# carefree0910/carefree-learn

Measured on AMD Instinct MI355X. Metric: train samples/sec + step ms, ViT-B/16 bf16 DDP at 1/2/4/8 MI355X, higher is better.
Workload: dtype bf16

## Files before the change

### __graft_entry__.py

```python
import os
import subprocess
import sys

ROOT = os.path.dirname(os.path.abspath(__file__))
if ROOT not in sys.path:
    sys.path.insert(0, ROOT)

CSRC = os.path.join(ROOT, "carefree-learn_amd", "csrc")
SOURCES = ["errors", "gemm", "gemm_grouped", "attn", "attn_wide", "attn_probs", "norm", "elementwise", "conv", "conv_grouped", "groupnorm", "embed", "random", "tabular", "comm", "sample", "lora", "vq", "conv_direct"]


def build() -> None:
    out_dir = os.path.join(ROOT, "carefree-learn_amd", "_build")
    os.makedirs(out_dir, exist_ok=True)
    hipcc = os.environ.get("HIPCC", "hipcc")
    flags = ["--offload-arch=gfx950", "-O3", "-std=c++17", "-fPIC", "-munsafe-fp-atomics"]
    procs = []
    for name in SOURCES:
        cmd = [hipcc, *flags, "-c", os.path.join(CSRC, name + ".hip"), "-o", os.path.join(out_dir, name + ".o")]
        procs.append((name, subprocess.Popen(cmd, cwd=CSRC)))
    for name, p in procs:
        if p.wait() != 0:
            raise RuntimeError(f"hipcc failed on {name}.hip")
    lib = os.path.join(ROOT, "carefree-learn_amd", "libcfhip.so")
# ... 57 lines not shown
```

### carefree-learn_amd/csrc/gemm.hip

```cpp
#include "gemm_device.h"

namespace {

template <bool AT, bool BT, class C>
struct ItemCtx {
  int m0, n0, z, klen, nk, tile_n;
  __amdgpu_buffer_rsrc_t a_rsrc, b_rsrc;
  StagePlan<C::A_INSTR> pa;
  StagePlan<C::B_INSTR> pb;
  unsigned yx[C::A_INSTR];
  int bshift[C::B_INSTR];
  int btap[C::B_INSTR];
  int kb;
};

template <bool AT, bool BT, class C, int CONV = 0>
__device__ __forceinline__ ItemCtx<AT, BT, C> setup_item(const GemmParams& p, int item, int wave, int lane) {
  ItemCtx<AT, BT, C> c;
  const int ntiles = p.tiles_m * p.tiles_n;
  c.z = item / ntiles;
  const int tile = item - c.z * ntiles;
  int tile_m;
  if (p.group_n > 0) {
    const int per_group = p.group_n * p.tiles_m;
// ... 612 lines not shown
  static const char* const cfg_names[NUM_CFG] = {
      "Cfg<128, 128, 2, 2, 2, 64>", "Cfg<128, 128, 2, 2, 2, 32>", "Cfg<128, 128, 2, 2, 3, 32>", "Cfg<128, 64, 2, 2, 2, 64>",
      "Cfg<128, 128, 2, 2, 4, 32>", "Cfg<128, 64, 2, 2, 2, 32>", "Cfg<128, 64, 2, 2, 3, 32>", "Cfg<256, 256, 2, 4, 4, 32>",
      "Cfg<256, 128, 2, 4, 3, 32>", "Cfg<256, 128, 2, 2, 3, 32>", "Cfg<128, 256, 2, 2, 3, 32>", "Cfg<256, 128, 2, 4, 6, 32>",
      "Cfg<256, 256, 2, 4, 5, 32>", "Cfg<256, 256, 2, 4, 2, 64>", "Cfg<192, 128, 2, 4, 2, 64>", "Cfg<192, 128, 2, 2, 2, 64>",
      "Cfg<128, 256, 2, 4, 2, 64>"};
  int epi = epilogue == CFHIP_EPI_QGELU ? CFHIP_EPI_GELU : epilogue == CFHIP_EPI_DQGELU ? CFHIP_EPI_DGELU : epilogue;
  int cfg = pick_config(M, N, a_trans, b_trans);
  cfg = resolve_config(cfg, a_trans, epi, false);
  const bool phase = cfg >= 7 && cfg <= 12;
  snprintf(out, out_bytes, "%s<%s, %s, %d, %s>", phase ? "gemm_bf16_phase_kernel" : "gemm_bf16_kernel",
           a_trans ? "true" : "false", b_trans ? "true" : "false", epi, cfg_names[cfg]);
  return CFHIP_OK;
}

extern "C" int cfhip_gemm_bf16(const void* A, const void* B, void* C, const float* bias,
                               const void* aux_in, void* aux_out, int M, int N, int K, int64_t lda,
                               int64_t ldb, int64_t ldc, int a_trans, int b_trans, int epilogue,
                               int out_dtype, int accumulate, int split_k, void* workspace,
                               size_t workspace_bytes, float* bias_grad, int bias_grad_accumulate,
                               void* stream) {
  CFHIP_REQUIRE(A && B && C, "gemm: null operand");
  CFHIP_REQUIRE(bias_grad == nullptr || (a_trans && b_trans),
                "gemm: the fused bias gradient exists for layout (1,1) only");
  CFHIP_REQUIRE(M > 0 && N > 0 && K > 0, "gemm: empty problem M=%d N=%d K=%d", M, N, K);
  CFHIP_REQUIRE(epilogue >= 0 && epilogue <= 5, "gemm: bad epilogue %d", epilogue);
  const int quick = epilogue == CFHIP_EPI_QGELU || epilogue == CFHIP_EPI_DQGELU;
  if (epilogue == CFHIP_EPI_QGELU) epilogue = CFHIP_EPI_GELU;
  if (epilogue == CFHIP_EPI_DQGELU) epilogue = CFHIP_EPI_DGELU;
  CFHIP_REQUIRE(!(epilogue == CFHIP_EPI_RESIDUAL || epilogue == CFHIP_EPI_DGELU) || aux_in,
                "gemm: epilogue %d needs aux_in", epilogue);
  CFHIP_REQUIRE(!accumulate || (out_dtype == 1 && epilogue == CFHIP_EPI_NONE), "gemm: accumulate needs f32 output and epilogue NONE");
  CFHIP_REQUIRE(!(epilogue == CFHIP_EPI_GELU || epilogue == CFHIP_EPI_DGELU) || out_dtype == 0,
                "gemm: the GELU / GELU' epilogues write bf16");
  CFHIP_REQUIRE(!(a_trans && !b_trans), "gemm: layout (a_trans=1, b_trans=0) is not provided");
  if (split_k < 1) split_k = 1;
// ... 45 lines not shown
    const int per = (steps + split_k - 1) / split_k;
    split_k = (steps + per - 1) / per;
    p.k_chunk = per * BK_MAX;
  }
  if (split_k > 1) {
    const size_t need = (size_t)split_k * M * N * sizeof(float) + (bias_grad ? (size_t)split_k * M * sizeof(float) : 0);
    if (workspace == nullptr || workspace_bytes < need) {
      cfhip_set_error("gemm: split_k=%d needs %zu workspace bytes, got %zu", split_k, need, workspace_bytes);
      return CFHIP_ERR_WORKSPACE;
    }
    p.slabs = reinterpret_cast<float*>(workspace);
    if (bias_grad) p.bgrad_slabs = p.slabs + (size_t)split_k * M * N;
  }

  int rc;
  int cfg = pick_config(M, N, a_trans, b_trans);
  cfg = resolve_config(cfg, a_trans, epilogue, bias_grad != nullptr);
  switch (cfg) {
    case 1: rc = launch_layout<CfgB>(p, a_trans, b_trans, epilogue, split_k, s); break;
    case 2: rc = launch_layout<CfgC>(p, a_trans, b_trans, epilogue, split_k, s); break;
    case 3: rc = launch_layout<CfgD>(p, a_trans, b_trans, epilogue, split_k, s); break;
    case 4: rc = launch_layout<CfgE>(p, a_trans, b_trans, epilogue, split_k, s); break;
    case 5: rc = launch_layout<CfgF>(p, a_trans, b_trans, epilogue, split_k, s); break;
    case 6: rc = launch_layout<CfgG>(p, a_trans, b_trans, epilogue, split_k, s); break;
    case 7: rc = launch_layout<CfgP, true>(p, a_trans, b_trans, epilogue, split_k, s); break;
    case 8: rc = launch_layout<CfgQ, true>(p, a_trans, b_trans, epilogue, split_k, s); break;
    case 9: rc = launch_layout<CfgR, true>(p, a_trans, b_trans, epilogue, split_k, s); break;
    case 10: rc = launch_layout<CfgS, true>(p, a_trans, b_trans, epilogue, split_k, s); break;
    case 11: rc = launch_layout<CfgT, true>(p, a_trans, b_trans, epilogue, split_k, s); break;
    case 12: rc = launch_layout<CfgU, true>(p, a_trans, b_trans, epilogue, split_k, s); break;
    case 13: rc = launch_layout<CfgW>(p, a_trans, b_trans, epilogue, split_k, s); break;
// ... 2 lines not shown
    case 16: rc = launch_layout<CfgV>(p, a_trans, b_trans, epilogue, split_k, s); break;
    default: rc = launch_layout<CfgA>(p, a_trans, b_trans, epilogue, split_k, s); break;
  }
  if (rc != CFHIP_OK) return rc;
  CFHIP_CHECK_LAUNCH("gemm_bf16");

  if (split_k > 1) {
    const long total = (long)M * (N / 4);
    int blocks = (int)((total + 255) / 256);
    if (blocks > 2048) blocks = 2048;
    hipLaunchKernelGGL(splitk_reduce_kernel, dim3(blocks), dim3(256), 0, s, p.slabs, C, bias, M, N,
                       (long)ldc, split_k, out_dtype, accumulate, p.bgrad_slabs, p.bgrad, p.bgrad_acc);
    CFHIP_CHECK_LAUNCH("splitk_reduce");
  }
  return CFHIP_OK;
}

template <class C, bool PIPE>
static int launch_conv(GemmParams p, int split_k, hipStream_t s) {
  p.tiles_m = (p.M + C::BM - 1) / C::BM;
  p.tiles_n = (p.N + C::BN - 1) / C::BN;
  p.splits = split_k;
  return launch_cfg<false, false, CFHIP_EPI_NONE, C, PIPE, 1>(p, dim3(p.tiles_m * p.tiles_n * split_k), s);
}

struct ConvPlan { int form, split; };

static int conv_split_for(long tiles, long slots, int Cin) {
  const int steps = (9 * Cin + BK_MAX - 1) / BK_MAX;
  if (tiles * 2 > slots || steps < 16) return 1;
// ... 161 lines not shown
```

### carefree-learn_amd/fused.py

```python
import os
from typing import Any, Optional

import torch
from torch import Tensor
from torch.autograd import Function

from . import functional as _functional
from . import ops
from .functional import SideStream, bf16, f32, claim_grads, claim_grads_one_flag, commit_grads, shadow_bf16


FUSE_BIAS_GRAD = True
_SKIP_BIAS_GRAD = False


def _dw_db(w: Tensor, b: Optional[Tensor], dy2: Tensor, x2: Tensor) -> None:
    n, k = w.shape[0], x2.shape[1]
    split = ops.pick_split_k(n, k, x2.shape[0])
    prms = [w] + ([b] if (b is not None and b.requires_grad) else [])
    (gw, acc_w), *bias_claim = claim_grads(prms)
    kw = {}
    if bias_claim:
        gb, acc_b = bias_claim[0]
        if _SKIP_BIAS_GRAD:
# ... 161 lines not shown
        commit_grads((w, b), notify)
        return dx

    if not SPLIT_LN_BWD:
        return param_grads(True)
    SideStream.run(param_grads, (dy2, x2, mean, rstd), lane=1)
    dx, _, _ = ops.layernorm_bwd(dy2, x2, gamma, mean, rstd, dx_add=dx_add, want_param_grads=False, dx_out=dx_out,
                                 dx_add_lo=dx_add_lo, dx_lo_out=dx_lo_out)
    return dx


FWD_HALVES = int(os.environ.get("CFHIP_FWD_HALVES", "2"))


def _block_fwd(x2: Tensor, prm: tuple, num_heads: int, eps1: float, eps2: float, bsz: int, t: int,
               keep_mask: Optional[Tensor], causal: bool, quick: bool = False, streams: Optional[list] = None):
    ln1_w, ln1_b, in_w, qkv_b, out_w, out_b, ln2_w, ln2_b, w1, b1, w2, b2 = prm
    d = x2.shape[1]
    fb = lambda p: None if p is None else p.detach().reshape(-1)
    in_w16, out_w16 = shadow_bf16(in_w), shadow_bf16(out_w)
    w1_16, w2_16 = shadow_bf16(w1), shadow_bf16(w2)
    m, dev = bsz * t, x2.device
    ff = w1.shape[0]
    E = lambda *shape, dt=bf16: torch.empty(shape, dtype=dt, device=dev)
    ln1, mean1, rstd1 = E(m, d), E(m, dt=f32), E(m, dt=f32)
    qkv, o2, lse = E(m, 3 * d), E(m, d), E(bsz, num_heads, t, dt=f32)
    x1 = E(m, d, dt=x2.dtype)
    ln2, mean2, rstd2 = E(m, d), E(m, dt=f32), E(m, dt=f32)
    pre, h, y = E(m, ff), E(m, ff), E(m, d, dt=x2.dtype)
    act = ops.EPI_QGELU if quick else ops.EPI_GELU
    g1, bt1, g2, bt2 = ln1_w.detach(), ln1_b.detach(), ln2_w.detach(), ln2_b.detach()

    def run(b0: int, b1_: int) -> None:
        r = slice(b0 * t, b1_ * t)
        nb = b1_ - b0
        km = None if keep_mask is None else keep_mask[b0:b1_] if keep_mask.shape[0] == bsz else keep_mask
        ops.layernorm_fwd(x2[r], g1, bt1, eps1, out=ln1[r], mean=mean1[r], rstd=rstd1[r])
        ops.gemm(ln1[r], in_w16, bias=fb(qkv_b), out=qkv[r])
        q3 = qkv[r].view(nb, t, 3 * d)
        ops.attn_fwd(q3[..., :d], q3[..., d:2 * d], q3[..., 2 * d:], num_heads, mask=km, causal=causal,
                     out=o2[r].view(nb, t, d), lse=lse[b0:b1_])
        ops.gemm(o2[r], out_w16, bias=fb(out_b), epilogue=ops.EPI_RESIDUAL, aux_in=x2[r], out=x1[r])
        ops.layernorm_fwd(x1[r], g2, bt2, eps2, out=ln2[r], mean=mean2[r], rstd=rstd2[r])
        ops.gemm(ln2[r], w1_16, bias=fb(b1), epilogue=act, aux_out=pre[r], out=h[r])
        ops.gemm(h[r], w2_16, bias=fb(b2), epilogue=ops.EPI_RESIDUAL, aux_in=x1[r], out=y[r])

    if not streams or len(streams) == 1 or bsz < 2 * len(streams):
        run(0, bsz)
    else:
        n = len(streams)
        cuts = _slice_cuts(bsz, n)
        for i, st in enumerate(streams):
            with _functional.on_stream(st):
                run(cuts[i], cuts[i + 1])
    saved = (x2, mean1, rstd1, ln1, qkv, o2, lse, x1, mean2, rstd2, ln2, pre, h, in_w16, out_w16, w1_16, w2_16)
    return y, saved
# ... 3 lines not shown

FIRST_SLICE_SHARE = 0.5


def _slice_cuts(bsz: int, n: int) -> list:
    if n == 2 and FIRST_SLICE_SHARE != 0.5:
        first = min(bsz - 1, max(1, int(round(bsz * FIRST_SLICE_SHARE))))
        return [0, first, bsz]
    return [bsz * i // n for i in range(n + 1)]


BWD_HALVES = int(os.environ.get("CFHIP_BWD_HALVES", "2"))
SideStream.lanes = min(4, max(SideStream.lanes, BWD_HALVES, FWD_HALVES - 1))


def _block_bwd(saved: tuple, prm: tuple, num_heads: int, bsz: int, t: int, keep_mask: Optional[Tensor],
               causal: bool, d2: Tensor, quick: bool = False, streams: Optional[list] = None) -> Tensor:
    x2, mean1, rstd1, ln1, qkv, o2, lse, x1, mean2, rstd2, ln2, pre, h, in_w16, out_w16, w1_16, w2_16 = saved
    ln1_w, ln1_b, in_w, qkv_b, out_w, out_b, ln2_w, ln2_b, w1, b1, w2, b2 = prm
    two = d2.dim() == 3
    d2_full = d2
    d2, d2_lo = (d2[0], d2[1]) if two else (d2, None)
    d = d2.shape[1]
    m = bsz * t
    E = lambda cols: torch.empty((m, cols), dtype=bf16, device=d2.device)
    dpre, dqkv = E(pre.shape[1]), E(3 * d)
    if two:
        dx1_full, dx_full = (torch.empty((2, m, d), dtype=bf16, device=d2.device) for _ in range(2))
        (dx1, dx1_lo), (dx, dx_lo) = (dx1_full[0], dx1_full[1]), (dx_full[0], dx_full[1])
    else:
        dx1, dx = E(d), E(d)
        dx1_lo = dx_lo = None
# ... 14 lines not shown
        km = None if keep_mask is None else keep_mask[b0:b1_] if keep_mask.shape[0] == bsz else keep_mask
        cur = _functional.cur_stream() if d2.is_cuda else None

        def ln(which: int, dy_, x_, w_, b_, mean_, rstd_, add_, out_, add_lo_=None, out_lo_=None) -> None:
            if _ln_defers(w_, b_, dy_):
                _ln_bwd(dy_, x_, w_, b_, mean_, rstd_, dx_add=add_, dx_out=out_, notify=last, dx_add_lo=add_lo_, dx_lo_out=out_lo_)
                return
            if ln_done[which] is not None:
                _functional.rec_wait_event(cur, ln_done[which])
            _ln_bwd(dy_, x_, w_, b_, mean_, rstd_, dx_add=add_, dx_out=out_, notify=last, dx_add_lo=add_lo_, dx_lo_out=out_lo_)
            if nsl > 1 and not last:
                ev = torch.cuda.Event()
                _functional.rec_record_event(ev, cur)
                ln_done[which] = ev

        ops.gemm(d2[r], w2_16, b_trans=True, epilogue=dact, aux_in=pre[r], out=dpre[r])
        dln2 = ops.gemm(dpre[r], w1_16, b_trans=True)
        ln(0, dln2, x1[r], ln2_w, ln2_b, mean2[r], rstd2[r], d2[r], dx1[r], None if d2_lo is None else d2_lo[r],
           None if dx1_lo is None else dx1_lo[r])
        d_o = ops.gemm(dx1[r], out_w16, b_trans=True)
        q3, dq3 = qkv3[b0:b1_], dqkv3[b0:b1_]
        ops.attn_bwd(q3[..., :d], q3[..., d:2 * d], q3[..., 2 * d:], o3[b0:b1_], d_o.view(nb, t, d), lse[b0:b1_], num_heads,
                     dq=dq3[..., :d], dk=dq3[..., d:2 * d], dv=dq3[..., 2 * d:], mask=km, causal=causal)
        dln1 = ops.gemm(dqkv[r], in_w16, b_trans=True)
        ln(1, dln1, x2[r], ln1_w, ln1_b, mean1[r], rstd1[r], dx1[r], dx[r], None if dx1_lo is None else dx1_lo[r],
           None if dx_lo is None else dx_lo[r])

    if nsl == 1:
        run(0)
    else:
        for i, st in enumerate(streams):
            with _functional.on_stream(st):
                run(i)
    _queue_dw(w2, b2, d2, h)
    _queue_dw(w1, b1, dpre, ln2)
    _queue_dw(out_w, out_b, dx1, o2)
    _queue_dw(in_w, qkv_b, dqkv, ln1)
    if two:
        SideStream.keep.append(d2_full)
    return dx_full


GRAD_STREAM_WORDS = int(os.environ.get("CFHIP_GRAD_STREAM_WORDS", "2"))


def _as_bf16_rows(dy: Tensor, rows: int, d: int, words: int = 1) -> Tensor:
    if words == 2:
        out = torch.empty((2, rows, d), dtype=bf16, device=dy.device)
        if dy.dtype == bf16:
            out[0].copy_(dy.contiguous().view(rows, d))
            out[1].zero_()
        else:
            ops.split_f32(dy.float().contiguous().view(rows, d), out[0], out[1])
        return out
    if dy.dtype != bf16:
        dy = ops.to_bf16(dy.float().contiguous())
    return dy.contiguous().view(rows, d)

# ... 166 lines not shown
    n_fresh = n = 0
    fp = 0
    for p in params:
        if p is None:
            continue
        g = p.grad
        if g is None or not p.requires_grad:
            return None
        n += 1
        n_fresh += 1 if getattr(p, "_cfhip_fresh", False) else 0
        fp = (fp * 1000003 + p.data_ptr() + 31 * g.data_ptr()) & 0xFFFFFFFFFFFFFFFF
    state = 1 if n_fresh == n else 0 if n_fresh == 0 else None
    return None if state is None else (state, fp)


def _plan_for(x: Tensor, metas: tuple, keep_mask: Optional[Tensor], causal: bool, params: tuple, training: bool) -> Optional[StackPlan]:
    from . import _lib

    if (not STACK_PLANS or not x.is_cuda or not training or ops.GEMM_TIMER is not None or ops.FLOP_COUNTER is not None
            or _lib.RECORDER is not None or torch.cuda.is_current_stream_capturing() or params[2] is None):
        return None
    state = _grad_state(params)
    if state is None:
        return None
    key = (tuple(x.shape), x.dtype, metas, causal, None if keep_mask is None else keep_mask.data_ptr(), FWD_HALVES, BWD_HALVES,
           DW_GROUP_BLOCKS, DW_GROUP_TILES, DW_TAIL_BLOCKS, DW_PEROP_TAIL, LN_REDUCE_ASIDE, DW_GROUP_ON_MAIN, FIRST_SLICE_SHARE, FUSE_BIAS_GRAD,
           ops.FORCE_SPLIT_K, tuple(id(cb) for cb in _functional.grad_ready_callbacks), x.requires_grad, GRAD_STREAM_WORDS, state)
    pid = id(params[0])
    plan = _plans.get(pid)
    if plan is None or plan.key != key or (plan.params_ref and plan.params_ref[0]() is not params[0]):
        if len(_plans) >= _PLAN_CACHE:
            _plan_conflicts.pop(next(iter(_plans)), None)
            _plans.pop(next(iter(_plans)))
        if plan is not None and plan.params_ref and plan.params_ref[0]() is not params[0]:
            _plan_conflicts.pop(pid, None)
        plan = _plans[pid] = StackPlan(key, params)
    return plan


class MixingStackFn(Function):

    @staticmethod
# ... 1 lines not shown
        m0 = metas[0]
        return int(m0[4]) if len(m0) > 4 and m0[4] else default

    @staticmethod
    def _slices_bwd(metas: tuple, default: int) -> int:
        m0 = metas[0]
        return int(m0[5]) if len(m0) > 5 and m0[5] else MixingStackFn._slices(metas, default)

    @staticmethod
    def _words(metas: tuple, x_is_f32: bool) -> int:
        m0 = metas[0]
        w = int(m0[6]) if len(m0) > 6 and m0[6] else GRAD_STREAM_WORDS
        return 2 if (w == 2 and x_is_f32) else 1

    @staticmethod
    def _forward_body(cur: Tensor, bsz: int, t: int, metas: tuple, keep_mask: Optional[Tensor], causal: bool, params: tuple):
        nblk = len(metas)
        all_saved = []
        streams = None
        FWD_HALVES = MixingStackFn._slices(metas, globals()["FWD_HALVES"])
        if FWD_HALVES > 1 and cur.is_cuda and bsz >= 2 * FWD_HALVES:
            for i in range(nblk):
                for j in (2, 4, 8, 10):
                    shadow_bf16(params[12 * i + j])
            main = _functional.cur_stream()
            streams = [main] + [SideStream.fork(lane) for lane in range(FWD_HALVES - 1)]
            if any(st is None for st in streams):
                streams = None
        for i, meta in enumerate(metas):
            num_heads, eps1, eps2 = meta[:3]
            quick = bool(meta[3]) if len(meta) > 3 else False
            cur, saved = _block_fwd(cur, params[12 * i:12 * i + 12], num_heads, eps1, eps2, bsz, t, keep_mask, causal,
                                    quick, streams)
            all_saved.extend(saved)
        if streams is not None:
            for st in streams[1:]:
                _functional.rec_wait_stream(_functional.cur_stream(), st)
        return cur, all_saved

    @staticmethod
    def forward(ctx: Any, x: Tensor, metas: tuple, keep_mask: Optional[Tensor], causal: bool,
                *params: Optional[Tensor]) -> Tensor:
        from . import _lib

        bsz, t, d = x.shape
        if x.dtype not in (bf16, f32):
            x = x.float()
        cur = x.contiguous().view(bsz * t, d)
        assert len(params) == 12 * len(metas)
        ctx.params = params
        ctx.meta = (bsz, t, d, metas, causal)
        ctx.words = MixingStackFn._words(metas, x.dtype == f32)
        ctx.plan = None
        plan = _plan_for(x, metas, keep_mask, causal, params, any(ctx.needs_input_grad))
        if plan is not None and plan.in_flight and not plan.disabled:
            pid = id(params[0])
            n = _plan_conflicts[pid] = _plan_conflicts.get(pid, 0) + 1
            plan = _plans[pid] = StackPlan(plan.key, params)
            if n > 2:
                plan.disabled = True
                if n == 3:
                    import warnings

                    warnings.warn("cfhip: a block stack is called again before the backward of its previous call, repeatedly: "
                                  "launch plans are off for this stack (normal launch path; results are the same)")
        if plan is not None and not plan.in_flight and not plan.disabled:
            plan.calls += 1
            plan.mask_tensor = keep_mask
# ... 6 lines not shown
                    plan.repoint(plan.x_sites, cur.data_ptr())
                    plan.x_now = cur.data_ptr()
                plan.x_live = cur
                _replay(plan.fwd if w_now == plan.w_ptr else plan.fwd_alt)
                plan.in_flight = True
                ctx.plan = plan
                ctx.plan_alt = w_now != plan.w_ptr
                return plan.y_out.detach().view(bsz, t, d)
            if plan.calls >= 2 and not plan.ready_fwd:
                plan.keep, plan.fwd, plan.bwd = [], [], []
                plan.w_ptr = w_now
                _lib.RECORDER = plan.fwd
                try:
                    with _KeepAllocations(plan.keep):
                        plan.x_in = cur
                        y, all_saved = MixingStackFn._forward_body(cur, bsz, t, metas, keep_mask, causal, params)
                finally:
                    _lib.RECORDER = None
                plan.y_out, plan.all_saved = y, all_saved
                plan.ready_fwd, plan.in_flight = True, True
                ctx.plan, ctx.plan_alt = plan, False
                return y.detach().view(bsz, t, d)
        y, all_saved = MixingStackFn._forward_body(cur, bsz, t, metas, keep_mask, causal, params)
        ctx.save_for_backward(*all_saved, keep_mask)
        return y.view(bsz, t, d)

    @staticmethod
    def _backward_body(all_saved: list, keep_mask: Optional[Tensor], bsz: int, t: int, metas: tuple, causal: bool, d2: Tensor,
                       params: tuple) -> Tensor:
        streams = None
        BWD_HALVES = MixingStackFn._slices_bwd(metas, globals()["BWD_HALVES"])
        if BWD_HALVES > 1 and d2.is_cuda and bsz >= 2 * BWD_HALVES:
            main = _functional.cur_stream()
            streams = [main] + [SideStream.fork(lane + 1) for lane in range(BWD_HALVES - 1)]
            if any(st is None for st in streams) or len({id(st) for st in streams}) != len(streams) or SideStream.get(0) in streams[1:]:
                streams = None
        _slice_streams[:] = streams[1:] if streams else []
        try:
            for i in range(len(metas) - 1, -1, -1):
                saved = tuple(all_saved[N_SAVED * i:N_SAVED * (i + 1)])
                quick = bool(metas[i][3]) if len(metas[i]) > 3 else False
                before = _pending_tiles()
                global _perop_now
                if i < DW_PEROP_TAIL and not _perop_now:
                    _flush_dw(tuple(_slice_streams))
                    _perop_now = True
                d2 = _block_bwd(saved, params[12 * i:12 * i + 12], metas[i][0], bsz, t, keep_mask, causal, d2, quick, streams)
                if DW_GROUP_BLOCKS > 0 and DW_GROUP_TILES > 0:
                    now = _pending_tiles()
                    if now + (now - before) > DW_GROUP_TILES or i <= DW_TAIL_BLOCKS:
                        _flush_dw(tuple(_slice_streams))
                elif DW_GROUP_BLOCKS > 0 and (len(metas) - i) % DW_GROUP_BLOCKS == 0:
                    _flush_dw(tuple(_slice_streams))
            _flush_dw(tuple(_slice_streams))
            if streams is not None:
                for st in streams[1:]:
                    _functional.rec_wait_stream(_functional.cur_stream(), st)
                SideStream.keep.append(d2)
            if d2.dim() == 3:
                d2 = ops.join_bf16x2(d2[0], d2[1])
        except BaseException:
            _pending_dw.clear()
# ... 2 lines not shown
            _slice_streams[:] = []
            _perop_now = False
        return d2

    @staticmethod
    def backward(ctx: Any, dy: Tensor):
        from . import _lib

        bsz, t, d, metas, causal = ctx.meta
        params = ctx.params
        plan: Optional[StackPlan] = ctx.plan
        nret = (None, None, None) + (None,) * len(params)
        if plan is None:
            *all_saved, keep_mask = ctx.saved_tensors
            d2 = _as_bf16_rows(dy, bsz * t, d, ctx.words)
            d2 = MixingStackFn._backward_body(list(all_saved), keep_mask, bsz, t, metas, causal, d2, params)
            return (d2.view(bsz, t, d),) + nret
        plan.in_flight = False
        if _plan_conflicts:
            _plan_conflicts.pop(id(params[0]), None)
        km = plan.mask_tensor
        fresh = _grad_state(params) == plan.state
        if plan.ready_bwd and fresh and _lib.RECORDER is None and ops.GEMM_TIMER is None and ops.FLOP_COUNTER is None:
            d2 = _as_bf16_rows(dy, bsz * t, d, ctx.words)
            if d2.data_ptr() != plan.dy_now:
                plan.repoint(plan.dy_sites, d2.data_ptr())
                plan.dy_now = d2.data_ptr()
            SideStream.queue_join()
            _replay(plan.bwd_alt if ctx.plan_alt else plan.bwd)
            SideStream.keep.append(d2)
            plan.x_live = None
            return (plan.dx_out.detach().view(bsz, t, d),) + nret
        if not plan.ready_bwd and fresh and _lib.RECORDER is None:
            d2 = _as_bf16_rows(dy, bsz * t, d, ctx.words)
            plan.dy_in = d2
            _lib.RECORDER = plan.bwd
            try:
                with _KeepAllocations(plan.keep):
                    dx = MixingStackFn._backward_body(plan.all_saved, km, bsz, t, metas, causal, d2, params)
            finally:
                _lib.RECORDER = None
            plan.dx_out = dx
            plan.keep.append(dx)
            plan.finish_recording(params)
            plan.ready_bwd = True
            return (dx.detach().view(bsz, t, d),) + nret
        d2 = _as_bf16_rows(dy, bsz * t, d, ctx.words)
        saved = list(plan.all_saved)
        if plan.x_live is not None:
            saved[0] = plan.x_live
            plan.x_live = None
        d2 = MixingStackFn._backward_body(saved, km, bsz, t, metas, causal, d2, params)
        return (d2.view(bsz, t, d),) + nret


def mixing_block(x: Tensor, *args: Any) -> Tensor:
    return MixingBlockFn.apply(x, *args)


def mixing_stack(x: Tensor, metas: tuple, keep_mask: Optional[Tensor], causal: bool, params: list) -> Tensor:
    return MixingStackFn.apply(x, metas, keep_mask, causal, *params)
```

### carefree-learn_amd/modules.py

```python
import math
import os
import sys
from typing import Any, Callable, Dict, List, NamedTuple, Optional, Sequence, Tuple

import torch
import torch.nn as nn
from torch import Tensor
from torch.nn import Module

from . import functional as HF
from . import fused
from . import ops
from .registry import (
    attentions,
    build_module,
    channel_mixers,
    decoders,
    encoders,
    generators,
    register_module,
    safe_execute,
    shallow_copy_dict,
    token_mixers,
    update_dict,
# ... 1150 lines not shown
        if self.head_token is not None:
            nn.init.trunc_normal_(self.head_token, std=0.02)
        self.apply(self._init_weights)

    @staticmethod
    def _init_weights(m: Module) -> None:
        if isinstance(m, nn.Linear):
            nn.init.trunc_normal_(m.weight, std=0.02)
            if m.bias is not None:
                nn.init.constant_(m.bias, 0.0)
        elif isinstance(m, nn.LayerNorm):
            nn.init.constant_(m.bias, 0.0)
            nn.init.constant_(m.weight, 1.0)

    fuse_stack = True

    def _head_ln(self) -> Module:
        return self.head_norm if self.head_norm is not None else self.head.norms[0]

    def post_process(self, net: Tensor) -> Tensor:
        if self.no_head_norm:
            return net[:, 0] if self.head_token is not None else net
        if self.head_token is not None:
            return self._head_ln()(net[:, 0])
        return self._head_ln()(net)

    def check_fused_token_assembly(self) -> None:
        drop = self.pos_encoding.pos_drop
        if drop is not None and self.training and 0.0 < drop.p < 1.0:
            raise NotImplementedError("positional_encoding_dropout > 0 is not provided by the fused token-assembly "
# ... 25 lines not shown
            net = self.embedding_dropout(net)
        return net

    def forward_tokens(self, tokens: Tensor, *, hw: Optional[Tuple[int, int]] = None,
                       deterministic: bool = False, causal: bool = False, mask: Optional[Tensor] = None,
                       clip_skip: int = 0, apply_head: bool = True) -> Tensor:
        net = tokens
        blocks = list(self.mixing_blocks)
        if clip_skip > 0:
            blocks = blocks[:len(blocks) - clip_skip]
        if (self.fuse_stack and len(blocks) > 1 and net.dim() == 3 and mask is None
                and all(b.use_fused and b._fusable() for b in blocks)):
            metas, params = [], []
            slices = getattr(self, "stack_slices", None)
            sf, sb = (slices, 0) if isinstance(slices, int) else (tuple(slices) + (0, 0))[:2] if slices else (0, 0)
            extra = (int(sf or 0), int(sb or 0), int(getattr(self, "grad_stream_words", 0) or 0))
            for b in blocks:
                metas.append(b.fused_meta() + extra)
                params.extend(b.fused_params())
            net = fused.mixing_stack(net, tuple(metas), None, causal, params)
        else:
            for block in blocks:
                net = block(net, hw, deterministic=deterministic, mask=mask, causal=causal)
        return self.post_process(net) if apply_head else net

    def forward(self, net: Tensor, *, hw: Optional[Tuple[int, int]] = None, hwp: Any = None,
                deterministic: bool = False) -> Tensor:
        return self.forward_tokens(self.pre_process(net, hwp=hwp, deterministic=deterministic), hw=hw,
                                   deterministic=deterministic)


# ... 410 lines not shown
            raise NotImplementedError("token-type embeddings / text dropout / text poolers are outside the hot path")
        self.img_size, self.context_length = img_size, context_length
        self.logit_scale = nn.Parameter(torch.tensor(math.log(1 / 0.07)))
        if not use_vision:
            self.vit = None
        else:
            self.vision_latent_dim = vision_latent_dim
            self.vit = ViTEncoder(
                img_size=img_size, patch_size=vision_patch_size, in_channels=in_channels,
                latent_dim=vision_latent_dim, to_patches_config={"bias": False}, num_layers=vision_num_layers,
                norm_kwargs={"eps": vision_norm_eps}, embedding_norm=LayerNorm(vision_latent_dim, vision_norm_eps),
                attention_kwargs={"num_heads": vision_num_heads},
                feedforward_kwargs={"activation": vision_feedforward_activation}, norm_after_head=True,
                output_dim=latent_dim,
            )
        if not use_text:
            self.token_embedding = self.token_type_embedding = self.text_transformer = None
            self.text_latent_dropout = self.text_projection = None
        else:
            self.text_num_layers, self.text_latent_dim = text_num_layers, text_latent_dim
            self.token_embedding = nn.Embedding(vocab_size, text_latent_dim, padding_idx=text_padding_idx)
            self.token_type_embedding = None
            self.text_transformer = TeTEncoder(
                text_latent_dim, context_length, use_triu_attn_mask=use_text_triu_attn_mask,
                num_layers=text_num_layers, dropout=text_dropout, norm_position=text_norm_position,
                norm_kwargs={"eps": text_norm_eps},
                embedding_norm=LayerNorm(text_latent_dim, text_norm_eps) if use_text_embedding_norm else None,
                embedding_dropout=text_embedding_dropout, attention_kwargs={"num_heads": text_num_heads},
                feedforward_kwargs={"activation": text_feedforward_activation}, head_pooler=text_head_pooler,
            )
# ... 1308 lines not shown
```

### carefree-learn_amd/ops.py

```python
import math
import os
from typing import List, Optional, Tuple

import ctypes

import torch
from torch import Tensor

from . import _lib

_H = _lib.DEFINES
EPI_NONE, EPI_GELU, EPI_RESIDUAL, EPI_DGELU, EPI_QGELU, EPI_DQGELU = (_H["CFHIP_EPI_" + e] for e in ("NONE", "GELU", "RESIDUAL", "DGELU", "QGELU", "DQGELU"))

bf16 = torch.bfloat16
f32 = torch.float32


_raw_stream = getattr(torch._C, "_cuda_getCurrentRawStream", None)
_raw_device = getattr(torch._C, "_cuda_getDevice", None)


def _stream() -> int:
    if _raw_stream is not None and _raw_device is not None:
        return _raw_stream(_raw_device())
# ... 73 lines not shown
    a: Tensor,
    b: Tensor,
    *,
    a_trans: bool = False,
    b_trans: bool = False,
    bias: Optional[Tensor] = None,
    epilogue: int = EPI_NONE,
    aux_in: Optional[Tensor] = None,
    aux_out: Optional[Tensor] = None,
    out: Optional[Tensor] = None,
    out_dtype: torch.dtype = bf16,
    accumulate: bool = False,
    split_k: int = 1,
    bias_grad: Optional[Tensor] = None,
    bias_grad_accumulate: bool = False,
) -> Tensor:
    if a.dtype is not bf16 or b.dtype is not bf16 or not a.is_cuda or not b.is_cuda:
        _need(a, bf16, "a")
        _need(b, bf16, "b")
    sha, shb, sta, stb = a.shape, b.shape, a.stride(), b.stride()
    if len(sha) != 2 or sta[1] != 1:
        _mat(a, "a")
    if len(shb) != 2 or stb[1] != 1:
        _mat(b, "b")
    lda, ldb = sta[0], stb[0]
    m, k = (sha[1], sha[0]) if a_trans else (sha[0], sha[1])
    n, kb = (shb[1], shb[0]) if b_trans else (shb[0], shb[1])
    if k != kb:
        raise ValueError(f"cfhip gemm: reduction dims differ ({k} vs {kb})")
    if out is None:
# ... 16 lines not shown
                    raise ValueError(f"cfhip gemm: `{nm}` must match the output layout")
    if bias_grad is not None:
        _need(bias_grad, f32, "bias_grad")
        if bias_grad.numel() != m or not bias_grad.is_contiguous():
            raise ValueError("cfhip gemm: bias_grad must be a contiguous f32 [M]")
    ws, ws_bytes = None, 0
    if split_k > 1:
        ws = torch.empty((split_k * m * (n + (1 if bias_grad is not None else 0)),), dtype=f32, device=a.device)
        ws_bytes = ws.numel() * 4
    if FLOP_COUNTER is not None:
        FLOP_COUNTER.flops["gemm"] += 2.0 * m * n * k
    timer = GEMM_TIMER
    if timer is not None:
        e0, e1 = torch.cuda.Event(enable_timing=True), torch.cuda.Event(enable_timing=True)
        e0.record()
    rc = _lib.load().cfhip_gemm_bf16(
        a.data_ptr(), b.data_ptr(), out.data_ptr(), _p(bias), _p(aux_in), _p(aux_out), m, n, k, lda,
        ldb, ldc, int(a_trans), int(b_trans), epilogue, 1 if odt is f32 else 0,
        int(accumulate), split_k, _p(ws), ws_bytes, _p(bias_grad), int(bias_grad_accumulate), _stream(),
    )
    _lib.check(rc, "gemm")
    if timer is not None:
        e1.record()
        layout = "tn" if a_trans else ("nn" if b_trans else "nt")
        timer.records.append(((layout, m, n, k, int(epilogue)), e0, e1))
    return out


def gemm_grouped_tn(problems: list) -> None:
    if not problems:
        return
    arr = (_lib.GemmProblem * len(problems))()
    flops = 0.0
    for i, (dy, x, out, acc, bg, bg_acc) in enumerate(problems):
        _need(dy, bf16, "dy")
# ... 395 lines not shown
            delta.data_ptr(), mp, dq.data_ptr(), dk.data_ptr(), dv.data_ptr(), b, num_heads, tq, tk, int(head_dim),
            q_sb, q_st, k_sb, k_st, o_sb, o_st, ms_b, ms_h, ms_q, float(scale), int(causal), int(parts),
            float(dropout_p), int(seed), int(offset), _stream(),
        )
    else:
        rc = _lib.load().cfhip_attn_bwd_dh(
            q.data_ptr(), k.data_ptr(), v.data_ptr(), o.data_ptr(), d_o.data_ptr(), lse.data_ptr(),
            delta.data_ptr(), mp, dq.data_ptr(), dk.data_ptr(), dv.data_ptr(), b, num_heads, tq, tk, int(head_dim),
            q_sb, q_st, k_sb, k_st, o_sb, o_st, ms_b, ms_h, ms_q, float(scale), int(causal), int(parts), _stream(),
        )
    _lib.check(rc, "attn_bwd")




def im2row(img: Tensor, patch: int) -> Tensor:
    if img.dtype not in (f32, bf16) or not img.is_cuda or not img.is_contiguous() or img.dim() != 4:
        raise ValueError("cfhip im2row: img must be a contiguous f32/bf16 [B, C, H, W] device tensor")
    b, c, hh, ww = img.shape
    rows = torch.empty((b * (hh // patch) * (ww // patch), c * patch * patch), dtype=bf16, device=img.device)
    rc = _lib.load().cfhip_im2row(img.data_ptr(), int(img.dtype == bf16), rows.data_ptr(), b, c, hh, ww,
                                  patch, _stream())
    _lib.check(rc, "im2row")
    return rows


def assemble_tokens_fwd(patches: Tensor, head_token: Tensor, pos: Tensor, b: int,
                        out_dtype: torch.dtype = f32) -> Tensor:
    _need(patches, bf16, "patches")
    _need(head_token, f32, "head_token")
# ... 1552 lines not shown
```

### include/cfhip.h

```cpp
#ifndef CFHIP_H
#define CFHIP_H

#include <stddef.h>
#include <stdint.h>

#ifdef __cplusplus
extern "C" {
#endif

#define CFHIP_VERSION 100

#define CFHIP_OK 0
#define CFHIP_ERR_INVALID (-1)
#define CFHIP_ERR_LAUNCH (-2)
#define CFHIP_ERR_WORKSPACE (-3)

int cfhip_version(void);
const char* cfhip_last_error(void);
int cfhip_set_option(const char* name, int value);

#define CFHIP_EPI_NONE 0
#define CFHIP_EPI_GELU 1
#define CFHIP_EPI_RESIDUAL 2
#define CFHIP_EPI_DGELU 3
// ... 316 lines not shown
int cfhip_comm_destroy(void* comm);
int cfhip_comm_count(void* comm, int* world, int* rank);
int cfhip_comm_allreduce(void* comm, void* buf, size_t count, int dtype, void* stream);
int cfhip_comm_allgather(void* comm, const void* send, void* recv, size_t count_per_rank, int dtype, void* stream);
int cfhip_comm_reduce_scatter(void* comm, const void* send, void* recv, size_t count_per_rank, int dtype, void* stream);
int cfhip_comm_broadcast(void* comm, void* buf, size_t count, int dtype, int root, void* stream);

int cfhip_conv2d_grouped_fwd(const void* x, const void* w, const float* bias, void* y, int B, int Cin, int H, int W, int Cout,
                             int kh, int kw, int stride, int pad, int dil, int groups, void* stream);
int cfhip_conv2d_grouped_bwd_input(const void* dy, const void* w, void* dx, int B, int Cin, int H, int W, int Cout, int kh,
                                   int kw, int stride, int pad, int dil, int groups, void* stream);
int cfhip_conv2d_grouped_bwd_weight(const void* dy, const void* x, float* dw, int accumulate, float* bias_grad,
                                    int bias_grad_accumulate, int B, int Cin, int H, int W, int Cout, int kh, int kw,
                                    int stride, int pad, int dil, int groups, void* stream);

#ifdef __cplusplus
}
#endif
#endif
```

Measured before the change: 7360.

## Compute only the head-token row through the last ViT block's post-attention path

In training, the last transformer block now runs the out-projection, LN2, the MLP GEMMs and their backward counterparts only on the head (class) token row of each sample, using strided row views. Only that token feeds the classifier, so the other rows are dead work. The remaining rows are zero-filled so later layernorm and attention backward see consistent buffers. A new gemm entry point lets the kernel config be chosen from the full row count rather than the reduced M. This saves roughly most of one block's MLP FLOPs in forward and backward, at the cost of extra zero-fill kernels and a more complex, path-specific code path.

```diff
diff --git a/__graft_entry__.py b/__graft_entry__.py
--- a/__graft_entry__.py
+++ b/__graft_entry__.py
@@ -7,7 +7,7 @@
     sys.path.insert(0, ROOT)
 
 CSRC = os.path.join(ROOT, "carefree-learn_amd", "csrc")
-SOURCES = ["errors", "gemm", "gemm_grouped", "attn", "attn_wide", "attn_probs", "norm", "elementwise", "conv", "conv_grouped", "groupnorm", "embed", "random", "tabular", "comm", "sample", "lora", "vq", "conv_direct"]
+SOURCES = ["errors", "gemm", "gemm_grouped", "attn", "attn_wide", "attn_probs", "norm", "elementwise", "conv", "conv_grouped", "groupnorm", "embed", "random", "tabular", "comm", "sample", "lora", "vq", "conv_direct", "head_tail"]
 
 
 def build() -> None:
diff --git a/carefree-learn_amd/csrc/gemm.hip b/carefree-learn_amd/csrc/gemm.hip
--- a/carefree-learn_amd/csrc/gemm.hip
+++ b/carefree-learn_amd/csrc/gemm.hip
@@ -650,12 +650,12 @@
   return CFHIP_OK;
 }
 
-extern "C" int cfhip_gemm_bf16(const void* A, const void* B, void* C, const float* bias,
-                               const void* aux_in, void* aux_out, int M, int N, int K, int64_t lda,
-                               int64_t ldb, int64_t ldc, int a_trans, int b_trans, int epilogue,
-                               int out_dtype, int accumulate, int split_k, void* workspace,
-                               size_t workspace_bytes, float* bias_grad, int bias_grad_accumulate,
-                               void* stream) {
+static int gemm_bf16_impl(const void* A, const void* B, void* C, const float* bias,
+                          const void* aux_in, void* aux_out, int M, int N, int K, int64_t lda,
+                          int64_t ldb, int64_t ldc, int a_trans, int b_trans, int epilogue,
+                          int out_dtype, int accumulate, int split_k, void* workspace,
+                          size_t workspace_bytes, float* bias_grad, int bias_grad_accumulate,
+                          void* stream, int config_rows) {
   CFHIP_REQUIRE(A && B && C, "gemm: null operand");
   CFHIP_REQUIRE(bias_grad == nullptr || (a_trans && b_trans),
                 "gemm: the fused bias gradient exists for layout (1,1) only");
@@ -731,7 +731,7 @@
   }
 
   int rc;
-  int cfg = pick_config(M, N, a_trans, b_trans);
+  int cfg = pick_config(config_rows > M ? config_rows : M, N, a_trans, b_trans);
   cfg = resolve_config(cfg, a_trans, epilogue, bias_grad != nullptr);
   switch (cfg) {
     case 1: rc = launch_layout<CfgB>(p, a_trans, b_trans, epilogue, split_k, s); break;
@@ -764,6 +764,24 @@
     CFHIP_CHECK_LAUNCH("splitk_reduce");
   }
   return CFHIP_OK;
+}
+
+extern "C" int cfhip_gemm_bf16(const void* A, const void* B, void* C, const float* bias,
+                               const void* aux_in, void* aux_out, int M, int N, int K, int64_t lda,
+                               int64_t ldb, int64_t ldc, int a_trans, int b_trans, int epilogue,
+                               int out_dtype, int accumulate, int split_k, void* workspace,
+                               size_t workspace_bytes, float* bias_grad, int bias_grad_accumulate,
+                               void* stream) {
+  return gemm_bf16_impl(A, B, C, bias, aux_in, aux_out, M, N, K, lda, ldb, ldc, a_trans, b_trans, epilogue, out_dtype, accumulate,
+                        split_k, workspace, workspace_bytes, bias_grad, bias_grad_accumulate, stream, 0);
+}
+
+extern "C" int cfhip_gemm_bf16_rows(const void* A, const void* B, void* C, const float* bias, const void* aux_in, void* aux_out,
+                                    int M, int N, int K, int64_t lda, int64_t ldb, int64_t ldc, int b_trans, int epilogue,
+                                    int out_dtype, int config_rows, void* stream) {
+  CFHIP_REQUIRE(config_rows >= M, "gemm_rows: config_rows = %d is less than M = %d", config_rows, M);
+  return gemm_bf16_impl(A, B, C, bias, aux_in, aux_out, M, N, K, lda, ldb, ldc, 0, b_trans, epilogue, out_dtype, 0, 1, nullptr, 0,
+                        nullptr, 0, stream, config_rows);
 }
 
 template <class C, bool PIPE>
diff --git a/carefree-learn_amd/csrc/head_tail.hip b/carefree-learn_amd/csrc/head_tail.hip
--- /dev/null
+++ b/carefree-learn_amd/csrc/head_tail.hip
@@ -0,0 +1,29 @@
+#include "common.h"
+
+namespace {
+
+typedef __attribute__((ext_vector_type(4))) unsigned int chunk16;
+
+__global__ void head_rows_zero_kernel(chunk16* __restrict__ dst, long total, int chunks, long stride) {
+  const long step = (long)gridDim.x * blockDim.x;
+  for (long i = blockIdx.x * (long)blockDim.x + threadIdx.x; i < total; i += step) {
+    const long row = i / chunks;
+    dst[row * stride + (i - row * chunks)] = chunk16{0u, 0u, 0u, 0u};
+  }
+}
+
+}
+
+extern "C" int cfhip_head_rows_zero(void* dst, int rows, int cols, int64_t row_stride, int elem_bytes, void* stream) {
+  CFHIP_REQUIRE(dst && rows > 0 && cols > 0 && (elem_bytes == 2 || elem_bytes == 4), "head_rows_zero: bad arguments");
+  const long row_bytes = (long)cols * elem_bytes, stride_bytes = (long)row_stride * elem_bytes;
+  CFHIP_REQUIRE(row_bytes % 16 == 0 && stride_bytes % 16 == 0 && stride_bytes >= row_bytes && ((uintptr_t)dst & 15) == 0,
+                "head_rows_zero: rows of %ld bytes, %ld apart, must be 16-byte multiples of a 16-byte aligned tensor", row_bytes, stride_bytes);
+  const int chunks = (int)(row_bytes / 16);
+  const long total = (long)rows * chunks;
+  const long blocks = (total + 255) / 256;
+  hipLaunchKernelGGL(head_rows_zero_kernel, dim3((unsigned)(blocks > 4096 ? 4096 : blocks)), dim3(256), 0, (hipStream_t)stream, (chunk16*)dst,
+                     total, chunks, stride_bytes / 16);
+  CFHIP_CHECK_LAUNCH("head_rows_zero");
+  return CFHIP_OK;
+}
diff --git a/carefree-learn_amd/fused.py b/carefree-learn_amd/fused.py
--- a/carefree-learn_amd/fused.py
+++ b/carefree-learn_amd/fused.py
@@ -199,7 +199,8 @@
 
 
 def _block_fwd(x2: Tensor, prm: tuple, num_heads: int, eps1: float, eps2: float, bsz: int, t: int,
-               keep_mask: Optional[Tensor], causal: bool, quick: bool = False, streams: Optional[list] = None):
+               keep_mask: Optional[Tensor], causal: bool, quick: bool = False, streams: Optional[list] = None,
+               head_only: bool = False):
     ln1_w, ln1_b, in_w, qkv_b, out_w, out_b, ln2_w, ln2_b, w1, b1, w2, b2 = prm
     d = x2.shape[1]
     fb = lambda p: None if p is None else p.detach().reshape(-1)
@@ -225,6 +226,17 @@
         q3 = qkv[r].view(nb, t, 3 * d)
         ops.attn_fwd(q3[..., :d], q3[..., d:2 * d], q3[..., 2 * d:], num_heads, mask=km, causal=causal,
                      out=o2[r].view(nb, t, d), lse=lse[b0:b1_])
+        if head_only:
+            rows = nb * t
+            hv = lambda u: u[r].view(nb, -1)[:, :u.shape[1]]
+            with _Unrecorded():
+                ops.head_rows_zero(x1[r], d)
+                ops.head_rows_zero(h[r], ff)
+            ops.gemm(hv(o2), out_w16, bias=fb(out_b), epilogue=ops.EPI_RESIDUAL, aux_in=hv(x2), out=hv(x1), config_rows=rows)
+            ops.layernorm_fwd(x1[r], g2, bt2, eps2, out=ln2[r], mean=mean2[r], rstd=rstd2[r])
+            ops.gemm(hv(ln2), w1_16, bias=fb(b1), epilogue=act, aux_out=hv(pre), out=hv(h), config_rows=rows)
+            ops.gemm(hv(h), w2_16, bias=fb(b2), epilogue=ops.EPI_RESIDUAL, aux_in=hv(x1), out=hv(y), config_rows=rows)
+            return
         ops.gemm(o2[r], out_w16, bias=fb(out_b), epilogue=ops.EPI_RESIDUAL, aux_in=x2[r], out=x1[r])
         ops.layernorm_fwd(x1[r], g2, bt2, eps2, out=ln2[r], mean=mean2[r], rstd=rstd2[r])
         ops.gemm(ln2[r], w1_16, bias=fb(b1), epilogue=act, aux_out=pre[r], out=h[r])
@@ -258,8 +270,21 @@
 SideStream.lanes = min(4, max(SideStream.lanes, BWD_HALVES, FWD_HALVES - 1))
 
 
+class _Unrecorded:
+
+    def __enter__(self) -> None:
+        from . import _lib
+
+        self.rec, _lib.RECORDER = _lib.RECORDER, None
+
+    def __exit__(self, *exc: Any) -> None:
+        from . import _lib
+
+        _lib.RECORDER = self.rec
+
+
 def _block_bwd(saved: tuple, prm: tuple, num_heads: int, bsz: int, t: int, keep_mask: Optional[Tensor],
-               causal: bool, d2: Tensor, quick: bool = False, streams: Optional[list] = None) -> Tensor:
+               causal: bool, d2: Tensor, quick: bool = False, streams: Optional[list] = None, head_only: bool = False) -> Tensor:
     x2, mean1, rstd1, ln1, qkv, o2, lse, x1, mean2, rstd2, ln2, pre, h, in_w16, out_w16, w1_16, w2_16 = saved
     ln1_w, ln1_b, in_w, qkv_b, out_w, out_b, ln2_w, ln2_b, w1, b1, w2, b2 = prm
     two = d2.dim() == 3
@@ -304,11 +329,26 @@
                 _functional.rec_record_event(ev, cur)
                 ln_done[which] = ev
 
-        ops.gemm(d2[r], w2_16, b_trans=True, epilogue=dact, aux_in=pre[r], out=dpre[r])
-        dln2 = ops.gemm(dpre[r], w1_16, b_trans=True)
+        if head_only:
+            rows = nb * t
+            hv = lambda u: u[r].view(nb, -1)[:, :u.shape[1]]
+            dln2, d_o = (torch.empty((rows, d), dtype=bf16, device=d2.device) for _ in range(2))
+            hv0 = lambda u: u.view(nb, -1)[:, :d]
+            with _Unrecorded():
+                ops.head_rows_zero(dpre[r], dpre.shape[1])
+                ops.head_rows_zero(dln2, d)
+                ops.head_rows_zero(d_o, d)
+            ops.gemm(hv(d2), w2_16, b_trans=True, epilogue=dact, aux_in=hv(pre), out=hv(dpre), config_rows=rows)
+            ops.gemm(hv(dpre), w1_16, b_trans=True, out=hv0(dln2), config_rows=rows)
+        else:
+            ops.gemm(d2[r], w2_16, b_trans=True, epilogue=dact, aux_in=pre[r], out=dpre[r])
+            dln2 = ops.gemm(dpre[r], w1_16, b_trans=True)
         ln(0, dln2, x1[r], ln2_w, ln2_b, mean2[r], rstd2[r], d2[r], dx1[r], None if d2_lo is None else d2_lo[r],
            None if dx1_lo is None else dx1_lo[r])
-        d_o = ops.gemm(dx1[r], out_w16, b_trans=True)
+        if head_only:
+            ops.gemm(hv(dx1), out_w16, b_trans=True, out=hv0(d_o), config_rows=rows)
+        else:
+            d_o = ops.gemm(dx1[r], out_w16, b_trans=True)
         q3, dq3 = qkv3[b0:b1_], dqkv3[b0:b1_]
         ops.attn_bwd(q3[..., :d], q3[..., d:2 * d], q3[..., 2 * d:], o3[b0:b1_], d_o.view(nb, t, d), lse[b0:b1_], num_heads,
                      dq=dq3[..., :d], dk=dq3[..., d:2 * d], dv=dq3[..., 2 * d:], mask=km, causal=causal)
@@ -332,6 +372,9 @@
 
 
 GRAD_STREAM_WORDS = int(os.environ.get("CFHIP_GRAD_STREAM_WORDS", "2"))
+
+HEAD_ONLY = os.environ.get("CFHIP_HEAD_ONLY", "1") != "0"
+HEAD_ONLY_MIN_ROWS = 1024
 
 
 def _as_bf16_rows(dy: Tensor, rows: int, d: int, words: int = 1) -> Tensor:
@@ -528,6 +571,13 @@
     return None if state is None else (state, fp)
 
 
+def _plan_key(x: Tensor, metas: tuple, keep_mask: Optional[Tensor], causal: bool, state: tuple) -> tuple:
+    return (tuple(x.shape), x.dtype, metas, causal, None if keep_mask is None else keep_mask.data_ptr(), FWD_HALVES, BWD_HALVES,
+            DW_GROUP_BLOCKS, DW_GROUP_TILES, DW_TAIL_BLOCKS, DW_PEROP_TAIL, LN_REDUCE_ASIDE, DW_GROUP_ON_MAIN, FIRST_SLICE_SHARE, FUSE_BIAS_GRAD,
+            ops.FORCE_SPLIT_K, tuple(id(cb) for cb in _functional.grad_ready_callbacks), x.requires_grad, GRAD_STREAM_WORDS, HEAD_ONLY,
+            HEAD_ONLY_MIN_ROWS, state)
+
+
 def _plan_for(x: Tensor, metas: tuple, keep_mask: Optional[Tensor], causal: bool, params: tuple, training: bool) -> Optional[StackPlan]:
     from . import _lib
 
@@ -537,9 +587,7 @@
     state = _grad_state(params)
     if state is None:
         return None
-    key = (tuple(x.shape), x.dtype, metas, causal, None if keep_mask is None else keep_mask.data_ptr(), FWD_HALVES, BWD_HALVES,
-           DW_GROUP_BLOCKS, DW_GROUP_TILES, DW_TAIL_BLOCKS, DW_PEROP_TAIL, LN_REDUCE_ASIDE, DW_GROUP_ON_MAIN, FIRST_SLICE_SHARE, FUSE_BIAS_GRAD,
-           ops.FORCE_SPLIT_K, tuple(id(cb) for cb in _functional.grad_ready_callbacks), x.requires_grad, GRAD_STREAM_WORDS, state)
+    key = _plan_key(x, metas, keep_mask, causal, state)
     pid = id(params[0])
     plan = _plans.get(pid)
     if plan is None or plan.key != key or (plan.params_ref and plan.params_ref[0]() is not params[0]):
@@ -571,7 +619,13 @@
         return 2 if (w == 2 and x_is_f32) else 1
 
     @staticmethod
-    def _forward_body(cur: Tensor, bsz: int, t: int, metas: tuple, keep_mask: Optional[Tensor], causal: bool, params: tuple):
+    def _head_only(metas: tuple, keep_mask: Optional[Tensor], causal: bool, training: bool, rows: int) -> bool:
+        m = metas[-1]
+        return bool(HEAD_ONLY and len(m) > 7 and m[7] and training and keep_mask is None and not causal and rows >= HEAD_ONLY_MIN_ROWS)
+
+    @staticmethod
+    def _forward_body(cur: Tensor, bsz: int, t: int, metas: tuple, keep_mask: Optional[Tensor], causal: bool, params: tuple,
+                      head_only: bool = False):
         nblk = len(metas)
         all_saved = []
         streams = None
@@ -588,7 +642,7 @@
             num_heads, eps1, eps2 = meta[:3]
             quick = bool(meta[3]) if len(meta) > 3 else False
             cur, saved = _block_fwd(cur, params[12 * i:12 * i + 12], num_heads, eps1, eps2, bsz, t, keep_mask, causal,
-                                    quick, streams)
+                                    quick, streams, head_only and i == nblk - 1)
             all_saved.extend(saved)
         if streams is not None:
             for st in streams[1:]:
@@ -609,6 +663,7 @@
         ctx.meta = (bsz, t, d, metas, causal)
         ctx.words = MixingStackFn._words(metas, x.dtype == f32)
         ctx.plan = None
+        ho = ctx.head_only = MixingStackFn._head_only(metas, keep_mask, causal, any(ctx.needs_input_grad), bsz * t)
         plan = _plan_for(x, metas, keep_mask, causal, params, any(ctx.needs_input_grad))
         if plan is not None and plan.in_flight and not plan.disabled:
             pid = id(params[0])
@@ -645,20 +700,20 @@
                 try:
                     with _KeepAllocations(plan.keep):
                         plan.x_in = cur
-                        y, all_saved = MixingStackFn._forward_body(cur, bsz, t, metas, keep_mask, causal, params)
+                        y, all_saved = MixingStackFn._forward_body(cur, bsz, t, metas, keep_mask, causal, params, ho)
                 finally:
                     _lib.RECORDER = None
                 plan.y_out, plan.all_saved = y, all_saved
                 plan.ready_fwd, plan.in_flight = True, True
                 ctx.plan, ctx.plan_alt = plan, False
                 return y.detach().view(bsz, t, d)
-        y, all_saved = MixingStackFn._forward_body(cur, bsz, t, metas, keep_mask, causal, params)
+        y, all_saved = MixingStackFn._forward_body(cur, bsz, t, metas, keep_mask, causal, params, ho)
         ctx.save_for_backward(*all_saved, keep_mask)
         return y.view(bsz, t, d)
 
     @staticmethod
     def _backward_body(all_saved: list, keep_mask: Optional[Tensor], bsz: int, t: int, metas: tuple, causal: bool, d2: Tensor,
-                       params: tuple) -> Tensor:
+                       params: tuple, head_only: bool = False) -> Tensor:
         streams = None
         BWD_HALVES = MixingStackFn._slices_bwd(metas, globals()["BWD_HALVES"])
         if BWD_HALVES > 1 and d2.is_cuda and bsz >= 2 * BWD_HALVES:
@@ -676,7 +731,8 @@
                 if i < DW_PEROP_TAIL and not _perop_now:
                     _flush_dw(tuple(_slice_streams))
                     _perop_now = True
-                d2 = _block_bwd(saved, params[12 * i:12 * i + 12], metas[i][0], bsz, t, keep_mask, causal, d2, quick, streams)
+                d2 = _block_bwd(saved, params[12 * i:12 * i + 12], metas[i][0], bsz, t, keep_mask, causal, d2, quick, streams,
+                                head_only and i == len(metas) - 1)
                 if DW_GROUP_BLOCKS > 0 and DW_GROUP_TILES > 0:
                     now = _pending_tiles()
                     if now + (now - before) > DW_GROUP_TILES or i <= DW_TAIL_BLOCKS:
@@ -709,7 +765,7 @@
         if plan is None:
             *all_saved, keep_mask = ctx.saved_tensors
             d2 = _as_bf16_rows(dy, bsz * t, d, ctx.words)
-            d2 = MixingStackFn._backward_body(list(all_saved), keep_mask, bsz, t, metas, causal, d2, params)
+            d2 = MixingStackFn._backward_body(list(all_saved), keep_mask, bsz, t, metas, causal, d2, params, ctx.head_only)
             return (d2.view(bsz, t, d),) + nret
         plan.in_flight = False
         if _plan_conflicts:
@@ -732,7 +788,7 @@
             _lib.RECORDER = plan.bwd
             try:
                 with _KeepAllocations(plan.keep):
-                    dx = MixingStackFn._backward_body(plan.all_saved, km, bsz, t, metas, causal, d2, params)
+                    dx = MixingStackFn._backward_body(plan.all_saved, km, bsz, t, metas, causal, d2, params, ctx.head_only)
             finally:
                 _lib.RECORDER = None
             plan.dx_out = dx
@@ -745,7 +801,7 @@
         if plan.x_live is not None:
             saved[0] = plan.x_live
             plan.x_live = None
-        d2 = MixingStackFn._backward_body(saved, km, bsz, t, metas, causal, d2, params)
+        d2 = MixingStackFn._backward_body(saved, km, bsz, t, metas, causal, d2, params, ctx.head_only)
         return (d2.view(bsz, t, d),) + nret
 
 
diff --git a/carefree-learn_amd/modules.py b/carefree-learn_amd/modules.py
--- a/carefree-learn_amd/modules.py
+++ b/carefree-learn_amd/modules.py
@@ -1188,6 +1188,7 @@
             nn.init.constant_(m.weight, 1.0)
 
     fuse_stack = True
+    head_only_tail = True
 
     def _head_ln(self) -> Module:
         return self.head_norm if self.head_norm is not None else self.head.norms[0]
@@ -1243,7 +1244,9 @@
             metas, params = [], []
             slices = getattr(self, "stack_slices", None)
             sf, sb = (slices, 0) if isinstance(slices, int) else (tuple(slices) + (0, 0))[:2] if slices else (0, 0)
-            extra = (int(sf or 0), int(sb or 0), int(getattr(self, "grad_stream_words", 0) or 0))
+            head_only = bool(apply_head and self.head_token is not None and clip_skip == 0 and not causal and self.head_only_tail
+                             and torch.is_grad_enabled())
+            extra = (int(sf or 0), int(sb or 0), int(getattr(self, "grad_stream_words", 0) or 0), head_only)
             for b in blocks:
                 metas.append(b.fused_meta() + extra)
                 params.extend(b.fused_params())
@@ -1684,6 +1687,7 @@
                 feedforward_kwargs={"activation": vision_feedforward_activation}, norm_after_head=True,
                 output_dim=latent_dim,
             )
+            self.vit.encoder.head_only_tail = False
         if not use_text:
             self.token_embedding = self.token_type_embedding = self.text_transformer = None
             self.text_latent_dropout = self.text_projection = None
diff --git a/carefree-learn_amd/ops.py b/carefree-learn_amd/ops.py
--- a/carefree-learn_amd/ops.py
+++ b/carefree-learn_amd/ops.py
@@ -111,6 +111,7 @@
     split_k: int = 1,
     bias_grad: Optional[Tensor] = None,
     bias_grad_accumulate: bool = False,
+    config_rows: int = 0,
 ) -> Tensor:
     if a.dtype is not bf16 or b.dtype is not bf16 or not a.is_cuda or not b.is_cuda:
         _need(a, bf16, "a")
@@ -157,11 +158,17 @@
     if timer is not None:
         e0, e1 = torch.cuda.Event(enable_timing=True), torch.cuda.Event(enable_timing=True)
         e0.record()
-    rc = _lib.load().cfhip_gemm_bf16(
-        a.data_ptr(), b.data_ptr(), out.data_ptr(), _p(bias), _p(aux_in), _p(aux_out), m, n, k, lda,
-        ldb, ldc, int(a_trans), int(b_trans), epilogue, 1 if odt is f32 else 0,
-        int(accumulate), split_k, _p(ws), ws_bytes, _p(bias_grad), int(bias_grad_accumulate), _stream(),
-    )
+    if config_rows:
+        if a_trans or split_k > 1 or accumulate or bias_grad is not None or config_rows < m:
+            raise ValueError("cfhip gemm: config_rows takes a_trans = False, no split_k / accumulate / bias_grad, and at least m rows")
+        rc = _lib.load().cfhip_gemm_bf16_rows(a.data_ptr(), b.data_ptr(), out.data_ptr(), _p(bias), _p(aux_in), _p(aux_out), m, n, k, lda,
+                                              ldb, ldc, int(b_trans), epilogue, 1 if odt is f32 else 0, int(config_rows), _stream())
+    else:
+        rc = _lib.load().cfhip_gemm_bf16(
+            a.data_ptr(), b.data_ptr(), out.data_ptr(), _p(bias), _p(aux_in), _p(aux_out), m, n, k, lda,
+            ldb, ldc, int(a_trans), int(b_trans), epilogue, 1 if odt is f32 else 0,
+            int(accumulate), split_k, _p(ws), ws_bytes, _p(bias_grad), int(bias_grad_accumulate), _stream(),
+        )
     _lib.check(rc, "gemm")
     if timer is not None:
         e1.record()
@@ -587,6 +594,19 @@
 
 
 
+def _rows16(t: Tensor, name: str) -> None:
+    if not t.is_cuda or t.dim() != 2 or t.stride(1) != 1 or (t.stride(0) * t.element_size()) % 16 or t.data_ptr() % 16:
+        raise ValueError(f"cfhip head tail: `{name}` must be a 2-D device tensor of 16-byte aligned rows")
+
+
+def head_rows_zero(x: Tensor, cols: int) -> None:
+    _rows16(x, "x")
+    rc = _lib.load().cfhip_head_rows_zero(x.data_ptr(), x.shape[0], cols, x.stride(0), x.element_size(), _stream())
+    _lib.check(rc, "head_rows_zero")
+
+
+
+
 def im2row(img: Tensor, patch: int) -> Tensor:
     if img.dtype not in (f32, bf16) or not img.is_cuda or not img.is_contiguous() or img.dim() != 4:
         raise ValueError("cfhip im2row: img must be a contiguous f32/bf16 [B, C, H, W] device tensor")
diff --git a/include/cfhip.h b/include/cfhip.h
--- a/include/cfhip.h
+++ b/include/cfhip.h
@@ -354,6 +354,11 @@
                                     int bias_grad_accumulate, int B, int Cin, int H, int W, int Cout, int kh, int kw,
                                     int stride, int pad, int dil, int groups, void* stream);
 
+int cfhip_gemm_bf16_rows(const void* A, const void* B, void* C, const float* bias, const void* aux_in, void* aux_out, int M, int N,
+                         int K, int64_t lda, int64_t ldb, int64_t ldc, int b_trans, int epilogue, int out_dtype, int config_rows,
+                         void* stream);
+int cfhip_head_rows_zero(void* dst, int rows, int cols, int64_t row_stride, int elem_bytes, void* stream);
+
 #ifdef __cplusplus
 }
 #endif
```

After: 7548, median of 6. 2.6% higher.
